# Priceincoding/nebula

Measured on AMD Instinct MI355X. Metric: GTEPS for GO 3 STEPS on RMAT-26 at 1/2/4/8 GPUs; % of HBM roofline, higher is better.
Workload: dtype int64; 1 GPU; GO 3 STEPS FROM 64 seeds OVER follow WHERE follow.weight > 499 YIELD DISTINCT follow._dst; RMAT-26 ef16; vertices=32803048, edges_after_collapse=1060378721, edges_scanned_per_query=1545132647, parallelism=1 GPU

## Files before the change

nebula_amd/csrc/bottom_up.hip:

```cpp
#include <algorithm>
#include <cstdio>
#include <cstdlib>
#include <mutex>
#include <string>
#include <unordered_map>
#include <vector>

#include "device_common.h"
#include "engine.h"
#include "expr_device.h"
#include "go_device.h"
#include "go_launch.h"
#include "qpred.h"
#include "query_common.h"

namespace nbg {

__global__ __launch_bounds__(1024) void k_reduce_partials(const unsigned long long* partials, int nblocks,
                                                          unsigned long long* out,
                                                          const unsigned long long* gate = nullptr) {
  if (gate && *gate == 0ull) return;
  __shared__ unsigned long long s[kSlots][16];
  unsigned long long a[kSlots];
#pragma unroll
  for (int k = 0; k < kSlots; k++) a[k] = 0;
// ... 498 lines not shown
    else
      tile(t, std::integral_constant<int, 2>{});
  }
  for (int64_t t = work_tiles + wave; t < ntiles; t += nwaves)
    if (lane < 2) {
      nbits[2 * t + lane] = 0ull;
      pbits[2 * t + lane] = 0ull;
    }
  if (lane != 0) nfound = npend = nwords = 0;
  unsigned long long acc64[8] = {nfound, 0, nwords, npend, 0, 0, 0, 0};
  if (atomic_sums) block_add_sums(acc64, 8, lds, partials, atomic_sums);
  else block_store_partials(acc64, 8, lds, partials);
}

constexpr int kLeanChunk = 8;
__device__ inline void load_chunk8(const int32_t* __restrict__ tcol, int64_t a, int64_t re, bool act,
                                   int32_t (&sv)[kLeanChunk]) {
  int4 x = make_int4(-1, -1, -1, -1), y = x;
  if (act) x = *reinterpret_cast<const int4*>(tcol + a);
  if (act && a + 4 < re) y = *reinterpret_cast<const int4*>(tcol + a + 4);
  sv[0] = x.x, sv[1] = x.y, sv[2] = x.z, sv[3] = x.w;
  sv[4] = y.x, sv[5] = y.y, sv[6] = y.z, sv[7] = y.w;
}
template <int PK, int W, int HUB, int REC>
__global__ __launch_bounds__(1024, 4) void k_bu_rest_lean(const unsigned long long* __restrict__ pbits, int64_t n,
                                                          const int64_t* __restrict__ trp,
                                                          const int32_t* __restrict__ tcol,
                                                          const uint32_t* __restrict__ fbits, uint32_t fb_bytes,
                                                          unsigned long long* nbits,
                                                          const uint32_t* __restrict__ odeg, FastArgs fp, QArgs q_arg,
                                                          unsigned long long* partials, int cw, int ru, int rest_from,
                                                          int steps, unsigned long long* dbg,
                                                          const unsigned long long* __restrict__ gate,
                                                          const uint4* __restrict__ rec, int atomic_sums) {
  if (gate && *gate == 0ull) return;
  const QArgs q = q_sgpr(q_arg);
  __shared__ unsigned long long lds[kSlots * 16];
  __shared__ unsigned long long s_found[16][64];
  extern __shared__ uint32_t s_fb[];
  const unsigned long long t_in = wall_clock64();
  if (HUB) hub_fill(s_fb, fbits, cw, false);
  const unsigned long long t_hub = wall_clock64();
  uint32_t d_rows = 0, d_batches = 0, d_steps = 0, d_scan = 0;
  unsigned long long t_scan = 0;
  const __amdgpu_buffer_rsrc_t fb_rs = __builtin_amdgcn_make_buffer_rsrc(
      const_cast<uint32_t*>(fbits), 0, int(__builtin_amdgcn_readfirstlane(fb_bytes)), 0x00020000);
  auto in_front = [&](int32_t g) -> bool {
    const int32_t wi = g >> 5;
    uint32_t w;
    if (HUB && wi < cw) w = s_fb[wi];
    else w = __builtin_amdgcn_raw_buffer_load_b32(fb_rs, wi * 4, 0, 0);
    return (w >> (g & 31)) & 1u;
  };
  uint32_t acc[6] = {0, 0, 0, 0, 0, 0};
  unsigned long long odsum = 0;
  const int lane = threadIdx.x & 63, wv = threadIdx.x >> 6;
  const int64_t nwords = (n + 63) / 64;
  const int64_t wave = (int64_t(blockIdx.x) * blockDim.x + threadIdx.x) >> 6;
  const int64_t nwaves = (int64_t(gridDim.x) * blockDim.x) >> 6;
  for (int64_t cbase = 0; cbase + wave < nwords; cbase += nwaves * 64) {
    const int64_t myw = cbase + int64_t(lane) * nwaves + wave;
    const unsigned long long pw = myw < nwords ? pbits[myw] : 0ull;
    s_found[wv][lane] = 0ull;
    uint32_t total;
    const uint32_t pre = wave_excl_scan(uint32_t(__popcll(pw)), total);
    for (uint32_t k0 = 0; k0 < total; k0 += 64) {
      const uint32_t p = k0 + uint32_t(lane);
      bool pend[1] = {p < total}, found[1] = {false};
      int64_t rb[1] = {0}, re[1] = {0};
      int wsel = 0;
#pragma unroll
      for (int st = 32; st > 0; st >>= 1) {
        const uint32_t pv = __shfl(pre, wsel + st);
        if (wsel + st < 64 && pv <= p) wsel += st;
      }
      const unsigned long long wbits = __shfl((long long)pw, wsel);
      const uint32_t kk = p - __shfl(pre, wsel);
      int bit = 0;
#pragma unroll
      for (int st = 32; st > 0; st >>= 1)
        if (uint32_t(__popcll(wbits & ((1ull << (bit + st)) - 1ull))) <= kk) bit += st;
      const int32_t r = int32_t((cbase + int64_t(wsel) * nwaves + wave) * 64 + bit);
      auto test_chunk = [&](const int32_t(&sv)[kLeanChunk], int64_t base, int64_t lo_e, int64_t hi_e, bool act,
                            bool count) __attribute__((always_inline)) -> bool {
        uint32_t w[kLeanChunk];
        int tq[kLeanChunk];
#pragma unroll
        for (int k = 0; k < kLeanChunk; k++) {
          const bool valid = act && base + k >= lo_e && base + k < hi_e;
          if (count) acc[4] += valid;
          tq[k] = PK == PK_FAST ? q_test(sv[k], q) : 1;
          const bool cand = valid && tq[k] != 0;
          const int32_t wi = q_gidx(sv[k], q) >> 5;
          const bool hub = HUB && wi < cw;
          const uint32_t gw = __builtin_amdgcn_raw_buffer_load_b32(fb_rs, cand && !hub ? uint32_t(wi) * 4u : 0xfffffff0u,
                                                                   0, 0);
          if (HUB) {
            const uint32_t lw = s_fb[cand && hub ? wi : 0];
            w[k] = cand && hub ? lw : gw;
          } else {
            w[k] = gw;
          }
        }
        __builtin_amdgcn_sched_barrier(0);
        bool h = false, need = false;
        uint32_t und = 0;
#pragma unroll
        for (int k = 0; k < kLeanChunk; k++) {
          const bool inf = (w[k] >> (uint32_t(sv[k]) & 31u)) & 1u;
          h = h || (inf && tq[k] > 0);
          if (PK == PK_FAST && inf && tq[k] < 0) {
            und |= 1u << k;
            need = true;
          }
        }
        if (PK == PK_FAST && __ballot(need && !h)) {
          if (!h) {
#pragma unroll
            for (int k = 0; k < kLeanChunk; k++)
              if ((und >> k) & 1u) {
                acc[5]++;
                h = h || fast_cmp(fp.op, load_w<W>(fp.data, fp.width, base + k), fp.k);
              }
          }
        }
        return h;
      };
      int64_t r0 = 0;
      if (REC) {
        uint4 x0 = make_uint4(0u, 0u, 0u, 0u), x1 = x0, x2 = x0, x3 = x0;
        if (pend[0]) {
          const uint4* rp = rec + size_t(r) * 4;
          x0 = rp[0], x1 = rp[1], x2 = rp[2], x3 = rp[3];
        }
        const int64_t start = int64_t(x0.x) | (int64_t(x0.y & 0xffffu) << 32);
        const uint32_t deg = x0.y >> 16;
        const int64_t rend = start + int64_t(deg < uint32_t(kRecEntries) ? deg : uint32_t(kRecEntries));
        r0 = start + rest_from;
        const int32_t sa[kLeanChunk] = {int32_t(x0.z), int32_t(x0.w), int32_t(x1.x), int32_t(x1.y),
                                        int32_t(x1.z), int32_t(x1.w), int32_t(x2.x), int32_t(x2.y)};
        bool h = test_chunk(sa, start, r0, rend, pend[0], false);
        if (__ballot(pend[0] && !h && deg > 8u)) {
          const int32_t sb[kLeanChunk] = {int32_t(x2.z), int32_t(x2.w), int32_t(x3.x), int32_t(x3.y),
                                          int32_t(x3.z), int32_t(x3.w), -1, -1};
          h = test_chunk(sb, start + 8, r0, rend, pend[0] && !h, false) || h;
        }
        if (h) found[0] = true;
        pend[0] = pend[0] && !h && deg > uint32_t(kRecEntries);
        if (pend[0]) {
          re[0] = deg < 65535u ? start + deg : trp[r + 1];
          r0 = start + kRecEntries;
          rb[0] = r0 & ~int64_t(3);
        }
      } else if (pend[0]) {
        r0 = trp[r] + rest_from;
        re[0] = trp[r + 1];
        rb[0] = r0 & ~int64_t(3);
        pend[0] = r0 < re[0];
      }
      d_batches++;
      d_rows += p < total;
      for (int step = 0; step < steps; step++) {
        if (__ballot(pend[0]) == 0) break;
        d_steps++;
        int32_t sv[kLeanChunk];
        load_chunk8(tcol, rb[0], re[0], pend[0], sv);
        __builtin_amdgcn_sched_barrier(0);
        const bool h = test_chunk(sv, rb[0], r0, re[0], pend[0], true);
        if (h) found[0] = true;
        rb[0] += kLeanChunk;
        pend[0] = pend[0] && !h && rb[0] < re[0];
      }
      const uint32_t a3 = acc[3];
      const unsigned long long ts0 = wall_clock64();
      bu_rest_scan<PK, W, 1>(pend, found, rb, re, tcol, fp, ru, acc, in_front, q);
      t_scan += wall_clock64() - ts0;
      d_scan += acc[3] - a3;
      acc[3] = a3;
      if (found[0]) {
        atomicOr(&s_found[wv][wsel], 1ull << (r & 63));
        acc[0]++;
        if (odeg) odsum += odeg[r];
      }
    }
    __builtin_amdgcn_wave_barrier();
    const unsigned long long fw = s_found[wv][lane];
    if (fw) nbits[myw] |= fw;
    __builtin_amdgcn_wave_barrier();
  }
  if (dbg) {
    const unsigned long long t_out = wall_clock64();
    uint32_t tr = d_rows, te = acc[4];
#pragma unroll
    for (int o = 32; o > 0; o >>= 1) tr += __shfl_xor(tr, o), te += __shfl_xor(te, o);
    if (lane == 0) {
      unsigned long long* d = dbg + wave * 8;
      d[0] = t_in, d[1] = t_hub, d[2] = t_out, d[3] = tr, d[4] = d_batches << 16 | d_steps, d[5] = d_scan, d[6] = te,
      d[7] = t_scan;
    }
  }
  unsigned long long acc64[6] = {acc[0], odsum, acc[2], acc[3], acc[4], acc[5]};
  if (atomic_sums) block_add_sums(acc64, 6, lds, partials, atomic_sums);
  else block_store_partials(acc64, 6, lds, partials);
}

template <int MODE, int U = 4, int NT = 0>
__global__ __launch_bounds__(1024) void k_bits_compact(const uint32_t* __restrict__ bits, int64_t n, int64_t lo,
                                                       const int64_t* __restrict__ vid_of, void* out,
                                                       unsigned long long* n_out,
                                                       const unsigned long long* gate = nullptr) {
  if (gate && *gate == 0ull) return;
  constexpr int kTileWords = 1024;
  __shared__ uint32_t sw[kTileWords];
  __shared__ uint32_t so[kTileWords];
  __shared__ uint32_t lds[16];
  __shared__ unsigned long long s_base;
  const int64_t nwords = (n + 31) / 32;
  const int64_t ntiles = (nwords + kTileWords - 1) / kTileWords;
  const int lane = threadIdx.x & 63;
  const int wv = threadIdx.x >> 6;
  for (int64_t t = blockIdx.x; t < ntiles; t += gridDim.x) {
    const int64_t w0 = t * kTileWords + int64_t(threadIdx.x);
    uint32_t x = w0 < nwords ? bits[w0] : 0u;
    if ((w0 + 1) * 32 > n && w0 < nwords) x &= (1u << uint32_t(n - w0 * 32)) - 1u;
// ... 62 lines not shown
  q.gbits = es.q_gbits;
  if (pk != PK_FAST || fcol != es.q_field) return q;
  return make_qargs_core(es.q_min, es.q_range, es.q_bits, es.q_gbits, fp.op, fp.k);
}

void launch_bits_list(Ctx& c, const uint32_t* bits, int64_t rows, int64_t lo, int32_t* out, unsigned long long* n_out) {
  k_bits_compact<0><<<grid_cap((rows + 31) / 32, 1024, 4096), 1024, 0, c.stream>>>(bits, rows, lo, nullptr, out, n_out);
}
void launch_bits_vids(Ctx& c, const uint32_t* bits, int64_t rows, int64_t lo, void* out, unsigned long long* n_out,
                      const unsigned long long* gate) {
  const int grid = grid_cap((rows + 31) / 32, 1024, 4096);
  k_bits_compact<1, 8, 1><<<grid, 1024, 0, c.stream>>>(bits, rows, lo, c.vid_of.as<int64_t>(), out, n_out, gate);
}

namespace {

template <typename Fn>
struct Named {
  Fn fn;
  const char* name;
};
#define NBG_K(...) {__VA_ARGS__, "nbg::" #__VA_ARGS__}
static_assert(PK_NONE == 0 && PK_FAST == 1, "the kernel tables index by pk and spell it as a number");

struct BuPlan {
  QArgs q;
  bool fast = false;
  int pk = PK_NONE;
  int rest_from = 4;
  int64_t ntiles = 0;
  int64_t work = 0;
  int cw = 0;
  int bs = 256, grid = 1;
  size_t shm = 0;
  uint32_t fb_bytes = 0;
  int probe_stats = 0;
  int atomic_sums = 0;
  int grid2 = 512;
  int W = 0;
  int rcw = 0, ru = 1, rsteps = 4;
  size_t rshm = 4;
  int64_t rest_rows = 0;
  bool use_rec = false;
};

BuPlan bu_plan(Ctx& c, const EdgeSpace& es, int pk, bool final, const FastArgs& fp, int fcol, bool hop_front,
               bool out_zero, int shards) {
  const Csr& tr = es.tr;
  if (pk != PK_NONE && pk != PK_FAST) throw Error(NBG_E_DEVICE, "bottom-up hop with a VM predicate");
  if (!es.pair_col[0].p) throw Error(NBG_E_DEVICE, "bottom-up hop without the quad slab");
  BuPlan p;
  p.fast = pk == PK_FAST || final;
  if (pk == PK_FAST) {
    p.q = make_qargs(es, c.opt("bu_qpred", 1) != 0 ? pk : PK_NONE, fcol, fp);
  } else {
    p.q = make_qargs(es, PK_NONE, -1, fp);
    if (p.fast) p.q.ulo = p.q.uhi = INT32_MAX, p.q.below = p.q.above = 1;
  }
  p.rest_from = pk == PK_FAST ? 0 : 4;
  p.pk = p.fast ? PK_FAST : PK_NONE;
  p.ntiles = (tr.n_rows + 127) / 128;
  p.work = std::min(p.ntiles, p.fast ? es.bu_in_tiles : es.bu_both_tiles);
  const int64_t waves = std::max<int64_t>(1, p.work);
  const int64_t fb_words = (c.n_global + 31) / 32;
  const int64_t hub_cap = std::max<int64_t>(0, c.opt("bu_hub_cap", 36 * 1024));
  p.cw = int(std::min<int64_t>(c.opt(p.fast ? "bu_lean_lds_kb_final" : "bu_lean_lds_kb", p.fast ? 72 : 64) * 256,
                               std::min<int64_t>({fb_words, int64_t(36 * 1024), hub_cap})));
  p.bs = p.cw > 0 ? 1024 : 256;
  p.grid = int(std::max<int64_t>(
      1, std::min<int64_t>((waves + p.bs / 64 - 1) / (p.bs / 64),
                           std::min<int64_t>(p.cw > 0 ? 512 : 2048, kAggBlocks / 2))));
  p.shm = size_t(p.cw + 1) * 4;
  p.fb_bytes = uint32_t(fb_words * 4);
  if (hop_front && !c.sharded && es.bu_both_tiles > 0)
    p.fb_bytes = uint32_t(std::min<int64_t>(p.fb_bytes, (es.bu_both_tiles * 128 + 31) / 32 * 4));
  p.probe_stats = int(c.opt("bu_probe_stats", 0));
  p.atomic_sums =
      c.opt("bu_atomic_sums", 1) != 0 && c.opt("bu_rest_dbg", 0) == 0 ? (out_zero ? std::max(shards, 1) : 1) : 0;
  p.ru = int(std::max<int64_t>(1, std::min<int64_t>(c.opt("bu_unroll", 1), kRestMax)));
  p.W = p.fast ? int(fp.width) : 0;
  p.rcw = int(std::min<int64_t>(c.opt(p.fast ? "bu_rest_lds_kb_final" : "bu_rest_lds_kb", 0) * 256,
                                std::min<int64_t>({fb_words, int64_t(36 * 1024), hub_cap})));
  p.rshm = size_t(std::max(p.rcw, 1)) * 4;
  p.rsteps = int(std::max<int64_t>(1, c.opt("bu_rest_steps", 4)));
  p.rest_rows = std::min(tr.n_rows, p.work * 128);
  p.use_rec = es.brec.p && es.brec_rows >= std::min(tr.n_rows, p.work * 128) && c.opt("bu_rec", 1) != 0;
  return p;
}

struct BuOut {
  unsigned long long* nb;
  unsigned long long* pbits;
  unsigned long long* partials;
  unsigned long long* gate;
};

void bu_first_pass(Ctx& c, const EdgeSpace& es, const BuPlan& p, const uint32_t* fb, const uint32_t* odeg,
                   const BuOut& o, const GateIn& gi, BuLaunch& L) {
  const uint2* lo = es.pair_col[0].as<uint2>();
  const uint2* hi = es.pair_col[1].as<uint2>();
  const int cw = p.cw;
  if (p.fast && !p.probe_stats && c.opt("bu_fin", 1) != 0) {
    using Fn = decltype(&k_bu_fin<0, 0>);
    static const Named<Fn> fin[4] = {NBG_K(k_bu_fin<0, 0>), NBG_K(k_bu_fin<1, 0>), NBG_K(k_bu_fin<0, 1>),
                                     NBG_K(k_bu_fin<1, 1>)};
    const FinArgs fa = fin_args(p.q);
    const bool cls1 = fin_cls1_ok(fa) && c.opt("bu_fin_cls", 1) != 0;
    const size_t fshm = size_t((cw + 2) & ~1) * 4 + size_t(kSlots) * 16 * 8;
    const uint32_t rest = p.fb_bytes > uint32_t(cw) * 4u ? p.fb_bytes - uint32_t(cw) * 4u : 0u;
    const int nt = int(c.opt("bu_fin_nt", 1) != 0);
    const uint32_t* wide = c.opt("bu_fin_narrow", 1) != 0 ? es.tile_wide.as<uint32_t>() : nullptr;
    if (wide) L.flag_bytes = uint64_t(p.work) / 8;
    const Named<Fn>& k = fin[(cls1 ? 1 : 0) | nt << 1];
    if (fshm > 48 * 1024) lds_limit(reinterpret_cast<const void*>(k.fn), fshm);
    k.fn<<<p.grid, p.bs, fshm, c.stream>>>(lo, hi, p.ntiles, p.work, fb, o.nb, o.pbits, fa, o.partials, cw, rest, o.gate,
                                           gi, p.atomic_sums, wide);
    L.k0 = k.name;
    return;
  }
  enum { kPlain, kHub, kPlainStats, kHubStats, kHubNt };
  using Fn = decltype(&k_bu_lean<0, 1, 0, 0, 0, 0>);
  static const Named<Fn> lean[2][5] = {
      {NBG_K(k_bu_lean<0, 1, 0, 0, 0, 0>), NBG_K(k_bu_lean<0, 1, 1, 0, 0, 0>), NBG_K(k_bu_lean<0, 1, 0, 1, 0, 0>),
       NBG_K(k_bu_lean<0, 1, 1, 1, 0, 0>), NBG_K(k_bu_lean<0, 1, 1, 0, 1, 3>)},
      {NBG_K(k_bu_lean<1, 1, 0, 0, 0, 0>), NBG_K(k_bu_lean<1, 1, 1, 0, 0, 0>), NBG_K(k_bu_lean<1, 1, 0, 1, 0, 0>),
       NBG_K(k_bu_lean<1, 1, 1, 1, 0, 0>), NBG_K(k_bu_lean<1, 1, 1, 0, 1, 3>)}};
  int sel = p.probe_stats ? (cw > 0 ? kHubStats : kPlainStats) : (cw > 0 ? kHub : kPlain);
  if (sel == kHub && (p.fast || es.odeg8.p)) sel = kHubNt;
  const Named<Fn>& k = lean[p.pk][sel];
  if (p.shm > 48 * 1024) lds_limit(reinterpret_cast<const void*>(k.fn), p.shm);
  k.fn<<<p.grid, p.bs, p.shm, c.stream>>>(lo, hi, p.ntiles, p.work, fb, p.fb_bytes, o.nb, o.pbits,
                                          p.fast ? nullptr : odeg, p.q, o.partials, cw, es.odeg8.as<uint8_t>(), o.gate,
                                          gi, p.atomic_sums);
  L.k0 = k.name;
  if (!p.fast) L.od_bytes = uint64_t(p.work) * 128u * (sel == kHubNt ? 1u : 4u);
}

void bu_rest_pass(Ctx& c, const EdgeSpace& es, const BuPlan& p, const uint32_t* fb, const uint32_t* odeg,
                  const FastArgs& fp, const BuOut& o, unsigned long long* dbg, BuLaunch& L) {
  using Fn = decltype(&k_bu_rest_lean<0, 0, 0, 0>);
#define NBG_REST_ROW(PKV, WV)                                                                     \
  {NBG_K(k_bu_rest_lean<PKV, WV, 0, 0>), NBG_K(k_bu_rest_lean<PKV, WV, 0, 1>), \
   NBG_K(k_bu_rest_lean<PKV, WV, 1, 0>), NBG_K(k_bu_rest_lean<PKV, WV, 1, 1>)}
  static const Named<Fn> rest_none[4] = NBG_REST_ROW(0, 0);
  static const Named<Fn> rest_fast[4][4] = {NBG_REST_ROW(1, 1), NBG_REST_ROW(1, 2), NBG_REST_ROW(1, 4),
                                            NBG_REST_ROW(1, 8)};
#undef NBG_REST_ROW
  const int wi = p.W == 1 ? 0 : p.W == 2 ? 1 : p.W == 4 ? 2 : 3;
  const Named<Fn>& k = (p.fast ? rest_fast[wi] : rest_none)[(p.rcw > 0 ? 2 : 0) | (p.use_rec ? 1 : 0)];
  const Csr& tr = es.tr;
  const int32_t* tc = p.q.gbits ? es.tcol_q.as<int32_t>() : tr.col.as<int32_t>();
  const uint4* rec = p.use_rec ? es.brec.as<uint4>() : nullptr;
  if (p.rshm > 48 * 1024) lds_limit(reinterpret_cast<const void*>(k.fn), p.rshm);
  k.fn<<<p.grid2, 1024, p.rshm, c.stream>>>(o.pbits, p.rest_rows, tr.row_ptr.as<int64_t>(), tc, fb, p.fb_bytes, o.nb,
                                            odeg, fp, p.q, p.atomic_sums ? o.partials : o.partials + p.grid, p.rcw, p.ru,
                                            p.rest_from, p.rsteps, dbg, o.gate, rec, p.atomic_sums);
  L.k1 = k.name;
  L.rest_rec = p.use_rec;
}
#undef NBG_K

void bu_rest_dbg_dump(Ctx& c, const unsigned long long* dbg, int pk, int grid2) {
  std::vector<unsigned long long> h(size_t(grid2) * 16 * 8);
  NBG_HIP(hipMemcpyAsync(h.data(), dbg, h.size() * 8, hipMemcpyDeviceToHost, c.stream));
  NBG_HIP(hipStreamSynchronize(c.stream));
  if (const char* fn = getenv("NBG_DBG_FILE")) {
    if (FILE* f = fopen(fn, "ab")) {
      const uint64_t hdr[2] = {uint64_t(pk), uint64_t(grid2) * 16};
      fwrite(hdr, 8, 2, f);
      fwrite(h.data(), 8, h.size(), f);
      fclose(f);
    }
  }
}

}

BuLaunch launch_bu_lean(Ctx& c, EdgeSpace& es, const uint32_t* fb, uint32_t* nbits, const uint32_t* odeg, int pk,
                        const FastArgs& fp, int fcol, unsigned long long* out, bool hop_front, unsigned long long* gate,
                        GateIn gi, bool out_zero, int shards) {
  const BuPlan p = bu_plan(c, es, pk, !odeg, fp, fcol, hop_front, out_zero, shards);
  c.ws_pend.ensure(size_t(p.ntiles * 2 + 2) * 8);
  const BuOut o{reinterpret_cast<unsigned long long*>(nbits), c.ws_pend.as<unsigned long long>(),
                p.atomic_sums ? out : c.ws_partials.as<unsigned long long>(), gate};
  if (p.atomic_sums && !out_zero) NBG_HIP(hipMemsetAsync(out, 0, 8 * 8, c.stream));
  BuLaunch L;
  bu_first_pass(c, es, p, fb, odeg, o, gi, L);
  NBG_HIP(hipGetLastError());
  L.ev_first = timing_event(c);
  DevBuf dbg_buf;
  unsigned long long* dbg = nullptr;
  if (c.opt("bu_rest_dbg", 0)) {
    dbg_buf.alloc(size_t(p.grid2) * 16 * 64);
    NBG_HIP(hipMemsetAsync(dbg_buf.p, 0, size_t(p.grid2) * 16 * 64, c.stream));
    dbg = dbg_buf.as<unsigned long long>();
  }
  bu_rest_pass(c, es, p, fb, odeg, fp, o, dbg, L);
  NBG_HIP(hipGetLastError());
  if (!p.atomic_sums) reduce_partials(c, o.partials, p.grid + p.grid2, out, gate);
  NBG_HIP(hipGetLastError());
  if (dbg) bu_rest_dbg_dump(c, dbg, p.pk, p.grid2);
  return L;
}

uint64_t bu_first_bytes(const unsigned long long* h, int64_t n_rows, uint64_t od_bytes) {
  return h[kHopSlabWords] * 4 + 3 * (uint64_t(n_rows) / 8) + od_bytes;
}
uint64_t bu_rest_bytes(const unsigned long long* h, int pred_width, bool rec) {
  return h[kHopPending] * (rec ? 64 : 16) + h[kHopEntries] * 4 + h[kHopValues] * uint64_t(pred_width);
}

}
```

nebula_amd/csrc/engine.h:

```cpp
#pragma once
#include <hip/hip_runtime.h>

#include <atomic>
#include <chrono>
#include <cstdint>
#include <cstdio>
#include <cstring>
#include <map>
#include <memory>
#include <mutex>
#include <stdexcept>
#include <string>
#include <vector>

#include "../../include/nebula_amd.h"

namespace nbg {

struct Error : std::runtime_error {
  int32_t code;
  Error(int32_t c, const std::string& m) : std::runtime_error(m), code(c) {}
};

#define NBG_HIP(x)                                                                        \
// ... 338 lines not shown
  double comm_ms = 0;
  uint64_t comm_bytes = 0;
  int32_t n_hops = 0;
  nbg_hop_stat hops[NBG_MAX_HOP_STATS] = {};
  int32_t host_waits = 0;
  int32_t spec_hops = 0;
  int32_t launches = 0;
  int32_t comm_calls = 0;
  uint64_t hop_bytes_mark = 0;
  void hop(int32_t mode, bool final_hop, double ms, const unsigned long long* c6, double kernel_ms = -1,
           uint64_t kernel_bytes = 0) {
    const uint64_t b = expand_bytes - hop_bytes_mark;
    hop_bytes_mark = expand_bytes;
    if (n_hops >= NBG_MAX_HOP_STATS) return;
    nbg_hop_stat& h = hops[n_hops++];
    h.mode = mode;
    h.final_hop = final_hop ? 1 : 0;
    h.ms = ms;
    h.bytes = b;
    for (int i = 0; i < 8; i++) h.c[i] = c6 ? c6[i] : 0;
    h.kernel_ms = kernel_ms < 0 ? ms : kernel_ms;
    h.kernel_bytes = kernel_ms < 0 ? b : kernel_bytes;
  }
  void name_last_hop(const std::string& k0, const std::string& k1 = "", const char* k2 = nullptr) {
    if (n_hops == 0 || n_hops > NBG_MAX_HOP_STATS) return;
    std::string s = k0;
    if (!k1.empty()) s += "; " + k1;
    if (k2) s += std::string("; ") + k2;
    nbg_hop_stat& h = hops[n_hops - 1];
    snprintf(h.kernels, sizeof h.kernels, "%s", s.c_str());
  }
};

constexpr size_t kHostStageBytes = size_t(1) << 20;

struct Ctx {
  int32_t device = 0, num_parts = 1, rank = 0, world = 1;
  bool sharded = false;
  hipStream_t stream = nullptr;
  std::mutex mu;
  std::string last_error;
  void* comm = nullptr;

  bool finalized = false;
  int64_t n_global = 0;
  int64_t n_vertices = 0;
  std::vector<int64_t> base;
  std::vector<int64_t> counts;
  DevBuf vid_of;
  DevBuf brank;
  DevBuf ht_keys, ht_vals;
// ... 186 lines not shown
```

nebula_amd/csrc/go_device.h:

```cpp
#pragma once
#include "device_common.h"
#include "engine.h"
#include "qpred.h"

namespace nbg {

constexpr int kThreads = 256;
constexpr int kItems = 8;
constexpr int kTile = kThreads * kItems;

__device__ inline QArgs q_sgpr(const QArgs& a) {
  QArgs r;
  r.gmask = __builtin_amdgcn_readfirstlane(a.gmask);
  r.gbits = __builtin_amdgcn_readfirstlane(a.gbits);
  r.ulo = __builtin_amdgcn_readfirstlane(a.ulo);
  r.uhi = __builtin_amdgcn_readfirstlane(a.uhi);
  r.below = __builtin_amdgcn_readfirstlane(a.below);
  r.above = __builtin_amdgcn_readfirstlane(a.above);
  return r;
}
__device__ inline int32_t q_gidx(int32_t s, const QArgs& q) { return s & int32_t(q.gmask); }

__device__ inline uint32_t wave_excl_scan(uint32_t x, uint32_t& total) {
  const int lane = threadIdx.x & 63;
  uint32_t v = x;
#pragma unroll
  for (int o = 1; o < 64; o <<= 1) {
    uint32_t y = __shfl_up(v, o);
    if (lane >= o) v += y;
  }
  total = __shfl(v, 63);
  return v - x;
}

constexpr int kAggBlocks = 8192;
constexpr int kSlots = 8;
constexpr int kRestMax = 2;

__device__ inline uint32_t block_excl_scan_u32(uint32_t x, uint32_t& total, uint32_t* lds) {
  uint32_t wt;
  uint32_t pre = wave_excl_scan(x, wt);
  const int w = threadIdx.x >> 6;
  if ((threadIdx.x & 63) == 0) lds[w] = wt;
  __syncthreads();
  uint32_t off = 0, tot = 0;
  for (int i = 0; i < int(blockDim.x >> 6); i++) {
    if (i < w) off += lds[i];
    tot += lds[i];
  }
  __syncthreads();
  total = tot;
// ... 107 lines not shown
```

nebula_amd/csrc/go_launch.h:

```cpp
#pragma once
#include <initializer_list>
#include <string>
#include <vector>

#include "engine.h"
#include "expr_device.h"
#include "go_device.h"
#include "query_common.h"

namespace nbg {

struct Counters {
  unsigned long long* d;
  unsigned long long* h;
};

struct ColOut {
  void* data;
  int32_t type;
  int64_t* len;
};
constexpr int kMaxYields = 16;
struct YieldArgs {
  int32_t ncols;
// ... 8 lines not shown
  Ctx& c;
  size_t a;
  explicit CommTimer(Ctx& cc) : c(cc), a(timing_event(cc)) {}
  ~CommTimer() {
    const size_t b = timing_event(c);
    if (a != ~size_t(0) && b != ~size_t(0)) c.tpend.push_back(Ctx::PendingTime{a, b, -1, 2});
  }
};

int64_t degree_scan(Ctx& c, const int32_t* F, int64_t nF, const Csr& csr, DevBuf& degbuf, int64_t known);
template <int MODE>
void launch_expand(Ctx& c, ExpandArgs a, int pk, const FastArgs& fp, const Program* dprog, const EvalEnv& env,
                   int64_t E, bool tile_rows_ready = false);

void reduce_partials(Ctx& c, const unsigned long long* partials, int nblocks, unsigned long long* out,
                     const unsigned long long* gate = nullptr);
QArgs make_qargs(const EdgeSpace& es, int pk, int fcol, const FastArgs& fp);
void launch_bits_list(Ctx& c, const uint32_t* bits, int64_t rows, int64_t lo, int32_t* out, unsigned long long* n_out);
void launch_bits_vids(Ctx& c, const uint32_t* bits, int64_t rows, int64_t lo, void* out, unsigned long long* n_out,
                      const unsigned long long* gate);
struct BuLaunch {
  size_t ev_first = kNoEvent;
  std::string k0, k1;
  bool rest_rec = false;
  uint64_t od_bytes = 0;
  uint64_t flag_bytes = 0;
};
BuLaunch launch_bu_lean(Ctx& c, EdgeSpace& es, const uint32_t* fb, uint32_t* nbits, const uint32_t* odeg, int pk,
                        const FastArgs& fp, int fcol, unsigned long long* out, bool hop_front,
                        unsigned long long* gate = nullptr, GateIn gi = GateIn{}, bool out_zero = false,
                        int shards = 1);
uint64_t bu_first_bytes(const unsigned long long* h, int64_t n_rows, uint64_t od_bytes);
uint64_t bu_rest_bytes(const unsigned long long* h, int pred_width, bool rec);

constexpr int kSmallStarts = 4096;
int64_t map_bytes(const Ctx& c);
void ensure_workspaces(Ctx& c, int64_t nF_cap);
void allsum(Ctx& c, int64_t* v, int n, unsigned long long* dscratch);
void dev_allsum(Ctx& c, const unsigned long long* K, std::initializer_list<int> idx, unsigned long long* dst);
const uint32_t* global_bits(Ctx& c, const uint32_t* owned);
const uint32_t* global_bits_cnt(Ctx& c, const uint32_t* owned, const unsigned long long* cnt, unsigned long long* all);
void exchange_marks(Ctx& c, uint8_t* map, uint32_t* owned_bits = nullptr, const uint32_t* odeg = nullptr,
                    unsigned long long* sums = nullptr);
void exchange_roots(Ctx& c, int32_t* root_next);
void launch_compact(Ctx& c, uint8_t* map, int64_t lo, int64_t n, const int64_t* row_ptr, const uint8_t* row_ok,
                    int require_deg, int32_t* out, uint16_t* bits, unsigned long long* Kd,
// ... 37 lines not shown
```

nebula_amd/csrc/traverse.hip:

```cpp
#include <algorithm>
#include <map>
#include <memory>
#include <string>
#include <vector>

#include "engine.h"
#include "expr_device.h"
#include "go_launch.h"
#include "program.h"
#include "qpred.h"
#include "query_common.h"
#include "rows.h"

namespace nbg {

namespace {

bool is_lone_dst(const std::vector<Program>& yields) {
  return yields.size() == 1 && yields[0].n == 1 && yields[0].ins[0].op == P_DST;
}
bool pred_runs_bottom_up(const FastPred& fpk, const FastArgs& fp, const EdgeSpace& es) {
  return fpk.kind == PK_NONE || (fpk.kind == PK_FAST && fp.present == nullptr &&
                                 es.tr.props.size() > size_t(fpk.col) && es.tr.props[size_t(fpk.col)].data.p);
}
// ... 372 lines not shown
      hb.alloc(c.host_pool, size_t(c.n_global + 64) * 8);
      return hb.p;
    }
    d.alloc(size_t(c.n_global + 64) * 8);
    return d.p;
  }

  template <typename Fn>
  BuLaunch timed_bu(int32_t hop, Fn launch) {
    const size_t ia = timing_event(c);
    BuLaunch L = launch();
    const size_t ib = timing_event(c);
    c.tpend.push_back(Ctx::PendingTime{ia, ib, hop, 0});
    c.tpend.push_back(Ctx::PendingTime{ia, L.ev_first, hop, 1});
    return L;
  }
  void record_bu_hop(const unsigned long long* h, const BuLaunch& L, bool final = false, int64_t out_rows = 0) {
    c.timing.expand_launches++;
    c.timing.bu_steps++;
    const int pw = final && fpk.kind == PK_FAST ? fp.width : 0;
    const uint64_t kb = bu_first_bytes(h, es.tr.n_rows, L.od_bytes + L.flag_bytes), hb = kb + bu_rest_bytes(h, pw, L.rest_rec);
    c.timing.expand_bytes += hb + (final ? uint64_t(es.tr.n_rows) / 8 + uint64_t(out_rows) * 16 : 0);
    c.timing.hop(1, final, 0.0, h, 0.0, kb);
    c.timing.name_last_hop(L.k0, L.k1, final ? "nbg::k_bits_compact<1, 8, 1>" : nullptr);
  }
  void adopt_bu(const unsigned long long* h, int64_t list_len, int64_t n_global, int64_t e_global) {
    std::swap(bitsA, bitsB);
    have_list = false;
    list_n = list_len;
    off_ready = false;
    E = int64_t(h[kHopDegSum]);
    E_known = E;
    nset_global = n_global;
    Eg = e_global;
  }
  void adopt_compaction(bool lazy, bool whole_space) {
    int64_t ng = int64_t(K.h[kCntSet]), eg = int64_t(K.h[kCntDegSum]);
    if (multi && !whole_space) {
      const unsigned long long* g = piggy_used ? K.h + kSpecBase + kSpecSumN : K.h + kCntGlobal;
      ng = int64_t(g[0]), eg = int64_t(g[1]);
    }
    nF = lazy ? 0 : int64_t(K.h[kCntList]);
    list_n = lazy ? int64_t(K.h[whole_space ? kCntOwnKept : kCntKept]) : -1;
    E = int64_t(K.h[whole_space ? kCntOwnDegSum : kCntDegSum]);
    E_known = E;
    nset_global = ng;
    Eg = eg;
// ... 183 lines not shown
    const size_t ia = timing_event(c);
    launch_rev_pull(c, es, rows, n_own, fb, final ? nullptr : D.deg, reinterpret_cast<unsigned long long*>(bitsB),
                    K.d + kCntUpto, ks);
    NBG_HIP(hipGetLastError());
    const size_t ik = timing_event(c);
    if (final) {
      launch_bits_vids(c, bitsB, n_own, lo, vout, K.d + kCntList, nullptr);
      NBG_HIP(hipGetLastError());
    }
    const size_t ib = final ? timing_event(c) : ik;
    c.tpend.push_back(Ctx::PendingTime{ia, ib, c.timing.n_hops, 0});
    c.tpend.push_back(Ctx::PendingTime{ia, ik, c.timing.n_hops, 1});
    if (multi && !final) dev_allsum(c, K.d, {kCntUpto, kCntUpto + 1}, K.d + kCntGlobal);
    fetch_counters(c, K.d, kCntUpto + 5, K.h, nullptr, ks);
    const unsigned long long* h = K.h + kCntUpto;
    const int64_t n_out = final ? int64_t(K.h[kCntList]) : 0;
    c.timing.expand_launches++;
    c.timing.bu_steps++;
    const uint64_t kb = uint64_t(rows) * (8 + (es.out.row_ok.p ? 1 : 0)) + h[3] * 4 + (final ? 0 : h[0] * 4) +
                        uint64_t(n_own) / 8;
    c.timing.expand_bytes += kb + (final ? uint64_t(n_own) / 8 + uint64_t(n_out) * 16 : 0);
    const unsigned long long hs[8] = {h[0], h[1], 0, h[4], h[3], 0, 0, 0};
    c.timing.hop(6, final, 0.0, hs, 0.0, kb);
    c.timing.name_last_hop("nbg::k_rev_pull", "", final ? "nbg::k_bits_compact<1, 8, 1>" : nullptr);
    return n_out;
  }
  void hop_rev_pull() {
    rev_pull(false, nullptr);
    const unsigned long long* h = K.h + kCntUpto;
    std::swap(bitsA, bitsB);
    have_list = false;
    list_n = int64_t(h[2]);
    off_ready = false;
    E = E_known = int64_t(h[1]);
    nset_global = multi ? int64_t(K.h[kCntGlobal]) : int64_t(h[0]);
    Eg = multi ? int64_t(K.h[kCntGlobal + 1]) : E;
  }

  void frontier_args() {
    a.F = F;
    a.nF = nF;
    a.off = c.ws_off.as<int64_t>();
  }
  void record_td_hop(bool final, double ms, int64_t n, int64_t e, int64_t rows_out = 0) {
    const unsigned long long hs[8] = {(unsigned long long)n, (unsigned long long)e, uint64_t(rows_out), 0, 0, 0, 0, 0};
    c.timing.hop(0, final, ms, hs);
  }
// ... 493 lines not shown
```

Before: 4138 GTEPS.

## Split bottom-up record test into separate kernel and size rest grid to residency

Adds a `k_bu_rec` kernel that tests the inline per-row adjacency records for all pending rows. It writes the rows still unresolved into a residual bitmap, so the lean rest kernel only walks long tails and skips reloading the record payload. This split is gated behind the `bu_rec_pass` option, which defaults to off. The rest kernel's grid is now capped by default to the number of blocks that can be resident at once, computed by an occupancy query and cached; this aims to avoid a tail of non-resident blocks. Test-chunk logic is factored into shared device helpers, and hop kernel naming is extended to list the extra kernel.

```diff
diff --git a/nebula_amd/csrc/bottom_up.hip b/nebula_amd/csrc/bottom_up.hip
--- a/nebula_amd/csrc/bottom_up.hip
+++ b/nebula_amd/csrc/bottom_up.hip
@@ -1,6 +1,7 @@
 #include <algorithm>
 #include <cstdio>
 #include <cstdlib>
+#include <map>
 #include <mutex>
 #include <string>
 #include <unordered_map>
@@ -545,6 +546,95 @@
   sv[0] = x.x, sv[1] = x.y, sv[2] = x.z, sv[3] = x.w;
   sv[4] = y.x, sv[5] = y.y, sv[6] = y.z, sv[7] = y.w;
 }
+__device__ __forceinline__ int32_t bu_pending_row(unsigned long long pw, uint32_t pre, uint32_t p, int64_t cbase,
+                                                  int64_t nwaves, int64_t wave, int& wsel) {
+  wsel = 0;
+#pragma unroll
+  for (int st = 32; st > 0; st >>= 1) {
+    const uint32_t pv = __shfl(pre, wsel + st);
+    if (wsel + st < 64 && pv <= p) wsel += st;
+  }
+  const unsigned long long wbits = __shfl((long long)pw, wsel);
+  const uint32_t kk = p - __shfl(pre, wsel);
+  int bit = 0;
+#pragma unroll
+  for (int st = 32; st > 0; st >>= 1)
+    if (uint32_t(__popcll(wbits & ((1ull << (bit + st)) - 1ull))) <= kk) bit += st;
+  return int32_t((cbase + int64_t(wsel) * nwaves + wave) * 64 + bit);
+}
+template <int PK, int W, int HUB, bool COUNT, bool SLIM>
+__device__ __forceinline__ bool bu_test_chunk(const int32_t (&sv)[8], int64_t base, int lo_k, int hi_k, bool act,
+                                              const QArgs& q, const __amdgpu_buffer_rsrc_t& fb_rs,
+                                              const uint32_t* s_fb, int cw, const FastArgs& fp, uint32_t& n_entries,
+                                              uint32_t& n_values) {
+  uint32_t w[8];
+  int tq[8];
+#pragma unroll
+  for (int k = 0; k < 8; k++) {
+    const bool valid = act && k >= lo_k && k < hi_k;
+    if (COUNT) n_entries += valid;
+    tq[k] = PK == PK_FAST ? q_test(sv[k], q) : 1;
+    const bool cand = valid && tq[k] != 0;
+    const int32_t wi = q_gidx(sv[k], q) >> 5;
+    const bool hub = HUB && wi < cw;
+    const uint32_t gw =
+        __builtin_amdgcn_raw_buffer_load_b32(fb_rs, cand && !hub ? uint32_t(wi) * 4u : 0xfffffff0u, 0, 0);
+    if (HUB) {
+      const uint32_t lw = s_fb[cand && hub ? wi : 0];
+      w[k] = cand && hub ? lw : gw;
+    } else {
+      w[k] = gw;
+    }
+  }
+  __builtin_amdgcn_sched_barrier(0);
+  bool h = false, need = false;
+  uint32_t und = 0;
+#pragma unroll
+  for (int k = 0; k < 8; k++) {
+    int32_t s = sv[k];
+    int t = tq[k];
+    if (SLIM && PK == PK_FAST) {
+      asm volatile("" : "+v"(s));
+      t = q_test(s, q);
+    }
+    const bool inf = (w[k] >> (uint32_t(s) & 31u)) & 1u;
+    h = h || (inf && t > 0);
+    if (PK == PK_FAST && inf && t < 0) {
+      und |= 1u << k;
+      need = true;
+    }
+  }
+  if (PK == PK_FAST && __ballot(need && !h)) {
+    if (!h) {
+#pragma unroll
+      for (int k = 0; k < 8; k++)
+        if ((und >> k) & 1u) {
+          n_values++;
+          h = h || fast_cmp(fp.op, load_w<W>(fp.data, fp.width, base + k), fp.k);
+        }
+    }
+  }
+  return h;
+}
+template <int PK, int W, int HUB, bool SLIM>
+__device__ __forceinline__ bool bu_test_record(const uint4& x0, const uint4& x1, const uint4& x2, const uint4& x3,
+                                               int64_t start, uint32_t deg, int rest_from, bool act, const QArgs& q,
+                                               const __amdgpu_buffer_rsrc_t& fb_rs, const uint32_t* s_fb, int cw,
+                                               const FastArgs& fp, uint32_t& n_values) {
+  const int nrec = int(deg < uint32_t(kRecEntries) ? deg : uint32_t(kRecEntries));
+  uint32_t none = 0;
+  const int32_t sa[8] = {int32_t(x0.z), int32_t(x0.w), int32_t(x1.x), int32_t(x1.y),
+                         int32_t(x1.z), int32_t(x1.w), int32_t(x2.x), int32_t(x2.y)};
+  bool h = bu_test_chunk<PK, W, HUB, false, SLIM>(sa, start, rest_from, nrec, act, q, fb_rs, s_fb, cw, fp, none, n_values);
+  if (__ballot(act && !h && deg > 8u)) {
+    const int32_t sb[8] = {int32_t(x2.z), int32_t(x2.w), int32_t(x3.x), int32_t(x3.y),
+                           int32_t(x3.z), int32_t(x3.w), -1,           -1};
+    h = bu_test_chunk<PK, W, HUB, false, SLIM>(sb, start + 8, rest_from - 8, nrec - 8, act && !h, q, fb_rs, s_fb, cw, fp,
+                                         none, n_values) ||
+        h;
+  }
+  return h;
+}
 template <int PK, int W, int HUB, int REC>
 __global__ __launch_bounds__(1024, 4) void k_bu_rest_lean(const unsigned long long* __restrict__ pbits, int64_t n,
                                                           const int64_t* __restrict__ trp,
@@ -555,7 +645,8 @@
                                                           unsigned long long* partials, int cw, int ru, int rest_from,
                                                           int steps, unsigned long long* dbg,
                                                           const unsigned long long* __restrict__ gate,
-                                                          const uint4* __restrict__ rec, int atomic_sums) {
+                                                          const uint4* __restrict__ rec, int atomic_sums,
+                                                          int rec_done) {
   if (gate && *gate == 0ull) return;
   const QArgs q = q_sgpr(q_arg);
   __shared__ unsigned long long lds[kSlots * 16];
@@ -591,83 +682,19 @@
       const uint32_t p = k0 + uint32_t(lane);
       bool pend[1] = {p < total}, found[1] = {false};
       int64_t rb[1] = {0}, re[1] = {0};
-      int wsel = 0;
-#pragma unroll
-      for (int st = 32; st > 0; st >>= 1) {
-        const uint32_t pv = __shfl(pre, wsel + st);
-        if (wsel + st < 64 && pv <= p) wsel += st;
-      }
-      const unsigned long long wbits = __shfl((long long)pw, wsel);
-      const uint32_t kk = p - __shfl(pre, wsel);
-      int bit = 0;
-#pragma unroll
-      for (int st = 32; st > 0; st >>= 1)
-        if (uint32_t(__popcll(wbits & ((1ull << (bit + st)) - 1ull))) <= kk) bit += st;
-      const int32_t r = int32_t((cbase + int64_t(wsel) * nwaves + wave) * 64 + bit);
-      auto test_chunk = [&](const int32_t(&sv)[kLeanChunk], int64_t base, int64_t lo_e, int64_t hi_e, bool act,
-                            bool count) __attribute__((always_inline)) -> bool {
-        uint32_t w[kLeanChunk];
-        int tq[kLeanChunk];
-#pragma unroll
-        for (int k = 0; k < kLeanChunk; k++) {
-          const bool valid = act && base + k >= lo_e && base + k < hi_e;
-          if (count) acc[4] += valid;
-          tq[k] = PK == PK_FAST ? q_test(sv[k], q) : 1;
-          const bool cand = valid && tq[k] != 0;
-          const int32_t wi = q_gidx(sv[k], q) >> 5;
-          const bool hub = HUB && wi < cw;
-          const uint32_t gw = __builtin_amdgcn_raw_buffer_load_b32(fb_rs, cand && !hub ? uint32_t(wi) * 4u : 0xfffffff0u,
-                                                                   0, 0);
-          if (HUB) {
-            const uint32_t lw = s_fb[cand && hub ? wi : 0];
-            w[k] = cand && hub ? lw : gw;
-          } else {
-            w[k] = gw;
-          }
-        }
-        __builtin_amdgcn_sched_barrier(0);
-        bool h = false, need = false;
-        uint32_t und = 0;
-#pragma unroll
-        for (int k = 0; k < kLeanChunk; k++) {
-          const bool inf = (w[k] >> (uint32_t(sv[k]) & 31u)) & 1u;
-          h = h || (inf && tq[k] > 0);
-          if (PK == PK_FAST && inf && tq[k] < 0) {
-            und |= 1u << k;
-            need = true;
-          }
-        }
-        if (PK == PK_FAST && __ballot(need && !h)) {
-          if (!h) {
-#pragma unroll
-            for (int k = 0; k < kLeanChunk; k++)
-              if ((und >> k) & 1u) {
-                acc[5]++;
-                h = h || fast_cmp(fp.op, load_w<W>(fp.data, fp.width, base + k), fp.k);
-              }
-          }
-        }
-        return h;
-      };
+      int wsel;
+      const int32_t r = bu_pending_row(pw, pre, p, cbase, nwaves, wave, wsel);
       int64_t r0 = 0;
       if (REC) {
         uint4 x0 = make_uint4(0u, 0u, 0u, 0u), x1 = x0, x2 = x0, x3 = x0;
-        if (pend[0]) {
-          const uint4* rp = rec + size_t(r) * 4;
-          x0 = rp[0], x1 = rp[1], x2 = rp[2], x3 = rp[3];
-        }
+        const uint4* rp = rec + size_t(r) * 4;
+        if (pend[0]) x0 = rp[0];
+        if (pend[0] && !rec_done) x1 = rp[1], x2 = rp[2], x3 = rp[3];
         const int64_t start = int64_t(x0.x) | (int64_t(x0.y & 0xffffu) << 32);
         const uint32_t deg = x0.y >> 16;
-        const int64_t rend = start + int64_t(deg < uint32_t(kRecEntries) ? deg : uint32_t(kRecEntries));
-        r0 = start + rest_from;
-        const int32_t sa[kLeanChunk] = {int32_t(x0.z), int32_t(x0.w), int32_t(x1.x), int32_t(x1.y),
-                                        int32_t(x1.z), int32_t(x1.w), int32_t(x2.x), int32_t(x2.y)};
-        bool h = test_chunk(sa, start, r0, rend, pend[0], false);
-        if (__ballot(pend[0] && !h && deg > 8u)) {
-          const int32_t sb[kLeanChunk] = {int32_t(x2.z), int32_t(x2.w), int32_t(x3.x), int32_t(x3.y),
-                                          int32_t(x3.z), int32_t(x3.w), -1, -1};
-          h = test_chunk(sb, start + 8, r0, rend, pend[0] && !h, false) || h;
-        }
+        bool h = false;
+        if (!rec_done)
+          h = bu_test_record<PK, W, HUB, false>(x0, x1, x2, x3, start, deg, rest_from, pend[0], q, fb_rs, s_fb, cw, fp, acc[5]);
         if (h) found[0] = true;
         pend[0] = pend[0] && !h && deg > uint32_t(kRecEntries);
         if (pend[0]) {
@@ -689,7 +716,8 @@
         int32_t sv[kLeanChunk];
         load_chunk8(tcol, rb[0], re[0], pend[0], sv);
         __builtin_amdgcn_sched_barrier(0);
-        const bool h = test_chunk(sv, rb[0], r0, re[0], pend[0], true);
+        const bool h = bu_test_chunk<PK, W, HUB, true, false>(sv, rb[0], int(r0 - rb[0]), int(std::min<int64_t>(re[0] - rb[0], 8)),
+                                                       pend[0], q, fb_rs, s_fb, cw, fp, acc[4], acc[5]);
         if (h) found[0] = true;
         rb[0] += kLeanChunk;
         pend[0] = pend[0] && !h && rb[0] < re[0];
@@ -723,6 +751,71 @@
     }
   }
   unsigned long long acc64[6] = {acc[0], odsum, acc[2], acc[3], acc[4], acc[5]};
+  if (atomic_sums) block_add_sums(acc64, 6, lds, partials, atomic_sums);
+  else block_store_partials(acc64, 6, lds, partials);
+}
+
+template <int PK, int W>
+__global__ __launch_bounds__(1024, 8) void k_bu_rec(const unsigned long long* __restrict__ pbits,
+                                                    unsigned long long* __restrict__ rbits, int64_t n,
+                                                    const uint32_t* __restrict__ fbits, uint32_t fb_bytes,
+                                                    unsigned long long* nbits, const uint32_t* __restrict__ odeg,
+                                                    FastArgs fp, QArgs q_arg, unsigned long long* partials,
+                                                    int rest_from, const unsigned long long* __restrict__ gate,
+                                                    const uint4* __restrict__ rec, int atomic_sums) {
+  if (gate && *gate == 0ull) return;
+  const QArgs q = q_sgpr(q_arg);
+  __shared__ unsigned long long lds[kSlots * 16];
+  __shared__ unsigned long long s_found[16][64];
+  __shared__ unsigned long long s_res[16][64];
+  const __amdgpu_buffer_rsrc_t fb_rs = __builtin_amdgcn_make_buffer_rsrc(
+      const_cast<uint32_t*>(fbits), 0, int(__builtin_amdgcn_readfirstlane(fb_bytes)), 0x00020000);
+  uint32_t nfound = 0, nvalues = 0;
+  unsigned long long odsum = 0;
+  const int lane_id = threadIdx.x & 63;
+  const int wv = int(__builtin_amdgcn_readfirstlane(threadIdx.x >> 6));
+  const int64_t nwords = (n + 63) / 64;
+  const int64_t wave =
+      int64_t(__builtin_amdgcn_readfirstlane(uint32_t((int64_t(blockIdx.x) * blockDim.x + threadIdx.x) >> 6)));
+  const int64_t nwaves = (int64_t(gridDim.x) * blockDim.x) >> 6;
+  for (int64_t cbase = 0; cbase + wave < nwords; cbase += nwaves * 64) {
+    int lane = lane_id;
+    asm volatile("" : "+v"(lane));
+    const int64_t myw = cbase + int64_t(lane) * nwaves + wave;
+    const unsigned long long pw = myw < nwords ? pbits[myw] : 0ull;
+    s_found[wv][lane] = 0ull;
+    s_res[wv][lane] = 0ull;
+    uint32_t total;
+    const uint32_t pre = wave_excl_scan(uint32_t(__popcll(pw)), total, lane);
+    for (uint32_t k0 = 0; k0 < total; k0 += 64) {
+      const uint32_t p = k0 + uint32_t(lane);
+      const bool act = p < total;
+      int wsel;
+      const int32_t r = bu_pending_row(pw, pre, p, cbase, nwaves, wave, wsel);
+      uint4 x0 = make_uint4(0u, 0u, 0u, 0u), x1 = x0, x2 = x0, x3 = x0;
+      if (act) {
+        const uint4* rp = rec + size_t(r) * 4;
+        x0 = rp[0], x1 = rp[1], x2 = rp[2], x3 = rp[3];
+      }
+      const int64_t start = int64_t(x0.x) | (int64_t(x0.y & 0xffffu) << 32);
+      const uint32_t deg = x0.y >> 16;
+      const bool h =
+          bu_test_record<PK, W, 0, true>(x0, x1, x2, x3, start, deg, rest_from, act, q, fb_rs, nullptr, 0, fp, nvalues);
+      if (h) {
+        atomicOr(&s_found[wv][wsel], 1ull << (r & 63));
+        nfound++;
+        if (odeg) odsum += odeg[r];
+      } else if (act && deg > uint32_t(kRecEntries)) {
+        atomicOr(&s_res[wv][wsel], 1ull << (r & 63));
+      }
+    }
+    __builtin_amdgcn_wave_barrier();
+    const unsigned long long fw = s_found[wv][lane];
+    if (fw) nbits[myw] |= fw;
+    if (myw < nwords) rbits[myw] = s_res[wv][lane];
+    __builtin_amdgcn_wave_barrier();
+  }
+  unsigned long long acc64[6] = {nfound, odsum, 0, 0, 0, nvalues};
   if (atomic_sums) block_add_sums(acc64, 6, lds, partials, atomic_sums);
   else block_store_partials(acc64, 6, lds, partials);
 }
@@ -831,6 +924,9 @@
 };
 #define NBG_K(...) {__VA_ARGS__, "nbg::" #__VA_ARGS__}
 static_assert(PK_NONE == 0 && PK_FAST == 1, "the kernel tables index by pk and spell it as a number");
+static_assert(sizeof("nbg::k_bu_lean<1, 1, 1, 0, 1, 3>; nbg::k_bu_rest_lean<1, 8, 1, 1>; nbg::k_bu_rec<1, 8>; "
+                     "nbg::k_bits_compact<1, 8, 1>") <= sizeof(nbg_hop_stat::kernels),
+              "nbg_hop_stat::kernels holds the longest kernel list of a hop");
 
 struct BuPlan {
   QArgs q;
@@ -851,6 +947,8 @@
   size_t rshm = 4;
   int64_t rest_rows = 0;
   bool use_rec = false;
+  bool rec_pass = false;
+  int rest_grid = 0;
 };
 
 BuPlan bu_plan(Ctx& c, const EdgeSpace& es, int pk, bool final, const FastArgs& fp, int fcol, bool hop_front,
@@ -894,12 +992,17 @@
   p.rsteps = int(std::max<int64_t>(1, c.opt("bu_rest_steps", 4)));
   p.rest_rows = std::min(tr.n_rows, p.work * 128);
   p.use_rec = es.brec.p && es.brec_rows >= std::min(tr.n_rows, p.work * 128) && c.opt("bu_rec", 1) != 0;
+  p.rec_pass = p.use_rec && p.rcw == 0 && c.opt("bu_rest_dbg", 0) == 0 && c.opt("bu_rec_pass", 0) != 0;
+  p.rest_grid = c.opt("bu_rest_dbg", 0) != 0
+                    ? p.grid2
+                    : int(std::max<int64_t>(0, std::min<int64_t>(c.opt("bu_rest_grid", 0), p.grid2)));
   return p;
 }
 
 struct BuOut {
   unsigned long long* nb;
   unsigned long long* pbits;
+  unsigned long long* rbits;
   unsigned long long* partials;
   unsigned long long* gate;
 };
@@ -945,7 +1048,25 @@
   if (!p.fast) L.od_bytes = uint64_t(p.work) * 128u * (sel == kHubNt ? 1u : 4u);
 }
 
-void bu_rest_pass(Ctx& c, const EdgeSpace& es, const BuPlan& p, const uint32_t* fb, const uint32_t* odeg,
+int resident_rest_grid(const void* kern, size_t shm, int cap) {
+  static std::mutex mu;
+  static std::map<std::pair<const void*, size_t>, int> cache;
+  std::lock_guard<std::mutex> lk(mu);
+  const auto key = std::make_pair(kern, shm);
+  auto it = cache.find(key);
+  if (it == cache.end()) {
+    int dev = 0, cus = 0, per = 0;
+    const bool ok = hipGetDevice(&dev) == hipSuccess &&
+                    hipDeviceGetAttribute(&cus, hipDeviceAttributeMultiprocessorCount, dev) == hipSuccess &&
+                    hipOccupancyMaxActiveBlocksPerMultiprocessor(&per, kern, 1024, shm) == hipSuccess && cus > 0 &&
+                    per > 0;
+    if (!ok) (void)hipGetLastError();
+    it = cache.emplace(key, ok ? cus * per : 0).first;
+  }
+  return it->second > 0 ? std::min(it->second, cap) : cap;
+}
+
+int bu_rest_pass(Ctx& c, const EdgeSpace& es, const BuPlan& p, const uint32_t* fb, const uint32_t* odeg,
                   const FastArgs& fp, const BuOut& o, unsigned long long* dbg, BuLaunch& L) {
   using Fn = decltype(&k_bu_rest_lean<0, 0, 0, 0>);
 #define NBG_REST_ROW(PKV, WV)                                                                     \
@@ -961,11 +1082,29 @@
   const int32_t* tc = p.q.gbits ? es.tcol_q.as<int32_t>() : tr.col.as<int32_t>();
   const uint4* rec = p.use_rec ? es.brec.as<uint4>() : nullptr;
   if (p.rshm > 48 * 1024) lds_limit(reinterpret_cast<const void*>(k.fn), p.rshm);
-  k.fn<<<p.grid2, 1024, p.rshm, c.stream>>>(o.pbits, p.rest_rows, tr.row_ptr.as<int64_t>(), tc, fb, p.fb_bytes, o.nb,
-                                            odeg, fp, p.q, p.atomic_sums ? o.partials : o.partials + p.grid, p.rcw, p.ru,
-                                            p.rest_from, p.rsteps, dbg, o.gate, rec, p.atomic_sums);
+  unsigned long long* part = p.atomic_sums ? o.partials : o.partials + p.grid;
+  int blocks = 0;
+  if (p.rec_pass) {
+    using RecFn = decltype(&k_bu_rec<0, 0>);
+    static const Named<RecFn> rec_none = NBG_K(k_bu_rec<0, 0>);
+    static const Named<RecFn> rec_fast[4] = {NBG_K(k_bu_rec<1, 1>), NBG_K(k_bu_rec<1, 2>), NBG_K(k_bu_rec<1, 4>),
+                                             NBG_K(k_bu_rec<1, 8>)};
+    const Named<RecFn>& kr = p.fast ? rec_fast[wi] : rec_none;
+    const int gr = resident_rest_grid(reinterpret_cast<const void*>(kr.fn), 0, p.grid2);
+    kr.fn<<<gr, 1024, 0, c.stream>>>(o.pbits, o.rbits, p.rest_rows, fb, p.fb_bytes, o.nb, odeg, fp, p.q, part,
+                                     p.rest_from, o.gate, rec, p.atomic_sums);
+    L.k_rec = kr.name;
+    if (!p.atomic_sums) part += gr;
+    blocks += gr;
+  }
+  const int g = p.rest_grid > 0 ? p.rest_grid : resident_rest_grid(reinterpret_cast<const void*>(k.fn), p.rshm, p.grid2);
+  blocks += g;
+  k.fn<<<g, 1024, p.rshm, c.stream>>>(p.rec_pass ? o.rbits : o.pbits, p.rest_rows, tr.row_ptr.as<int64_t>(), tc, fb,
+                                            p.fb_bytes, o.nb, odeg, fp, p.q, part, p.rcw, p.ru, p.rest_from, p.rsteps, dbg,
+                                            o.gate, rec, p.atomic_sums, p.rec_pass ? 1 : 0);
   L.k1 = k.name;
   L.rest_rec = p.use_rec;
+  return blocks;
 }
 #undef NBG_K
 
@@ -989,8 +1128,10 @@
                         const FastArgs& fp, int fcol, unsigned long long* out, bool hop_front, unsigned long long* gate,
                         GateIn gi, bool out_zero, int shards) {
   const BuPlan p = bu_plan(c, es, pk, !odeg, fp, fcol, hop_front, out_zero, shards);
-  c.ws_pend.ensure(size_t(p.ntiles * 2 + 2) * 8);
+  const size_t pend_words = size_t(p.ntiles * 2 + 2);
+  c.ws_pend.ensure(pend_words * 2 * 8);
   const BuOut o{reinterpret_cast<unsigned long long*>(nbits), c.ws_pend.as<unsigned long long>(),
+                c.ws_pend.as<unsigned long long>() + pend_words,
                 p.atomic_sums ? out : c.ws_partials.as<unsigned long long>(), gate};
   if (p.atomic_sums && !out_zero) NBG_HIP(hipMemsetAsync(out, 0, 8 * 8, c.stream));
   BuLaunch L;
@@ -1004,9 +1145,9 @@
     NBG_HIP(hipMemsetAsync(dbg_buf.p, 0, size_t(p.grid2) * 16 * 64, c.stream));
     dbg = dbg_buf.as<unsigned long long>();
   }
-  bu_rest_pass(c, es, p, fb, odeg, fp, o, dbg, L);
+  const int rest_blocks = bu_rest_pass(c, es, p, fb, odeg, fp, o, dbg, L);
   NBG_HIP(hipGetLastError());
-  if (!p.atomic_sums) reduce_partials(c, o.partials, p.grid + p.grid2, out, gate);
+  if (!p.atomic_sums) reduce_partials(c, o.partials, p.grid + rest_blocks, out, gate);
   NBG_HIP(hipGetLastError());
   if (dbg) bu_rest_dbg_dump(c, dbg, p.pk, p.grid2);
   return L;
diff --git a/nebula_amd/csrc/engine.h b/nebula_amd/csrc/engine.h
--- a/nebula_amd/csrc/engine.h
+++ b/nebula_amd/csrc/engine.h
@@ -384,11 +384,13 @@
     h.kernel_ms = kernel_ms < 0 ? ms : kernel_ms;
     h.kernel_bytes = kernel_ms < 0 ? b : kernel_bytes;
   }
-  void name_last_hop(const std::string& k0, const std::string& k1 = "", const char* k2 = nullptr) {
+  void name_last_hop(const std::string& k0, const std::string& k1 = "", const std::string& k2 = "",
+                     const char* k3 = nullptr) {
     if (n_hops == 0 || n_hops > NBG_MAX_HOP_STATS) return;
     std::string s = k0;
     if (!k1.empty()) s += "; " + k1;
-    if (k2) s += std::string("; ") + k2;
+    if (!k2.empty()) s += "; " + k2;
+    if (k3) s += std::string("; ") + k3;
     nbg_hop_stat& h = hops[n_hops - 1];
     snprintf(h.kernels, sizeof h.kernels, "%s", s.c_str());
   }
diff --git a/nebula_amd/csrc/go_device.h b/nebula_amd/csrc/go_device.h
--- a/nebula_amd/csrc/go_device.h
+++ b/nebula_amd/csrc/go_device.h
@@ -27,6 +27,16 @@
 #pragma unroll
   for (int o = 1; o < 64; o <<= 1) {
     uint32_t y = __shfl_up(v, o);
+    if (lane >= o) v += y;
+  }
+  total = __shfl(v, 63);
+  return v - x;
+}
+__device__ inline uint32_t wave_excl_scan(uint32_t x, uint32_t& total, int lane) {
+  uint32_t v = x;
+#pragma unroll
+  for (int o = 1; o < 64; o <<= 1) {
+    uint32_t y = __shfl(v, (lane - o) & 63);
     if (lane >= o) v += y;
   }
   total = __shfl(v, 63);
diff --git a/nebula_amd/csrc/go_launch.h b/nebula_amd/csrc/go_launch.h
--- a/nebula_amd/csrc/go_launch.h
+++ b/nebula_amd/csrc/go_launch.h
@@ -54,6 +54,7 @@
 struct BuLaunch {
   size_t ev_first = kNoEvent;
   std::string k0, k1;
+  std::string k_rec;
   bool rest_rec = false;
   uint64_t od_bytes = 0;
   uint64_t flag_bytes = 0;
diff --git a/nebula_amd/csrc/traverse.hip b/nebula_amd/csrc/traverse.hip
--- a/nebula_amd/csrc/traverse.hip
+++ b/nebula_amd/csrc/traverse.hip
@@ -418,7 +418,7 @@
     const uint64_t kb = bu_first_bytes(h, es.tr.n_rows, L.od_bytes + L.flag_bytes), hb = kb + bu_rest_bytes(h, pw, L.rest_rec);
     c.timing.expand_bytes += hb + (final ? uint64_t(es.tr.n_rows) / 8 + uint64_t(out_rows) * 16 : 0);
     c.timing.hop(1, final, 0.0, h, 0.0, kb);
-    c.timing.name_last_hop(L.k0, L.k1, final ? "nbg::k_bits_compact<1, 8, 1>" : nullptr);
+    c.timing.name_last_hop(L.k0, L.k1, L.k_rec, final ? "nbg::k_bits_compact<1, 8, 1>" : nullptr);
   }
   void adopt_bu(const unsigned long long* h, int64_t list_len, int64_t n_global, int64_t e_global) {
     std::swap(bitsA, bitsB);
@@ -648,7 +648,7 @@
     c.timing.expand_bytes += kb + (final ? uint64_t(n_own) / 8 + uint64_t(n_out) * 16 : 0);
     const unsigned long long hs[8] = {h[0], h[1], 0, h[4], h[3], 0, 0, 0};
     c.timing.hop(6, final, 0.0, hs, 0.0, kb);
-    c.timing.name_last_hop("nbg::k_rev_pull", "", final ? "nbg::k_bits_compact<1, 8, 1>" : nullptr);
+    c.timing.name_last_hop("nbg::k_rev_pull", "", "", final ? "nbg::k_bits_compact<1, 8, 1>" : nullptr);
     return n_out;
   }
   void hop_rev_pull() {
```

Result: no change. 4127 GTEPS (-0.3%).
